# mjayantkumar/spark-timeseries

Measured on AMD Instinct MI355X. Metric: series-elements/sec + % HBM roofline (fill+lag+ACF) at 1/2/4/8 MI355X, higher is better.
Workload: dtype f64; 1 GPU; C3 shard: fill('linear') + autocorr(60), 12,500 series x 982,800 steps per GPU (N=8 -> C3's 100k x 982,800, 786 GB); series_per_gpu=12500, numLags=60, fill=linear, parallelism=dp1 (series sharded by key, one process per GPU)

## Files before the change

spark-timeseries_amd/csrc/sts_internal.hpp:

```cpp
#pragma once
#include <hip/hip_runtime.h>

#include <cstdint>
#include <cstdlib>

#include "sts.h"

namespace sts {

constexpr int kHB = 64;
constexpr int kHA = 128;
constexpr int kPartStride = 68;
constexpr int kPartSum = 64, kPartSq = 65, kPartShift = 66;
constexpr int kAcfEdge = 64;
constexpr bool kShortPairDefault = false;

struct TileArgs {
    const double* in;
    double* out;
    double* lagmat;
    double* partials;
    int32_t* err;
    int64_t S, T, ld_in, ld_out;
    int64_t tiles_per_series;
    int64_t tiles_per_chunk;
    int64_t chunks_per_series;
    int K;
    int max_lag;
    int include_original;
    double* acf_fused;
    const double* shift;
    int err_all;
};

struct FinalizeArgs {
    const double* F;
    const double* partials;
    double* acf;
    int64_t S, T, ldF, parts_per_series;
    int K;
    int32_t* exact;
};

#ifdef STS_AB
inline const char* ab_knob(const char* name) { return std::getenv(name); }
#else
inline const char* ab_knob(const char*) { return nullptr; }
#endif

int series_status(const int32_t* h, int64_t S, const char* what);
int set_error(int status, const char* msg);
int validate_call(int (*fn)(void*), void* ctx);
template <class F>
int validate(F&& f) {
    return validate_call([](void* c) { return (*static_cast<F*>(c))(); }, static_cast<void*>(&f));
}

hipError_t launch_tile(int method, int tw, const TileArgs& a, hipStream_t st);
hipError_t launch_acf_finalize(const FinalizeArgs& a, hipStream_t st);
hipError_t launch_acf_exact(const double* F, int64_t S, int64_t T, int64_t ldF, int K, const int32_t* exact,
                            double* acf, hipStream_t st);
hipError_t launch_acf_shift(const double* in, int64_t S, int64_t T, int64_t ld, int method, double* shift,
                            hipStream_t st);
constexpr int kFusedMaxLags = 63;
size_t acf_wide_partials(int64_t S, int64_t T, int K);
hipError_t launch_acf_wide(const double* F, int64_t S, int64_t T, int64_t ld, const double* shift, int K, double* part,
                           double* acf, int32_t* exact, hipStream_t st);

constexpr int kSegW = 512;
constexpr int kSegTiles = 128;
int seg_nt(int K);
hipError_t launch_segment(int method, const TileArgs& a, hipStream_t st);
bool short_ok(int method, int64_t T, int K);
hipError_t launch_short(int method, const TileArgs& a, hipStream_t st, bool pair);

int64_t spline_batch(int64_t S, int64_t T);
hipError_t launch_spline(const double* in, double* out, int64_t S, int64_t T, int64_t ld_in, int64_t ld_out,
                         int32_t* err, double* scratch, int64_t batch, hipStream_t st);

hipError_t launch_diff(const double* in, double* out, int64_t S, int64_t T, int64_t ld_in,
                       int64_t ld_out, int lag, int start, hipStream_t st);
hipError_t launch_diff_inplace(double* x, int64_t S, int64_t T, int64_t ld, int lag, int start,
                               hipStream_t st);
hipError_t launch_lagmat(const double* in, double* out, int64_t S, int64_t T, int64_t ld_in,
                         int max_lag, int include_original, hipStream_t st);
hipError_t launch_ewma_remove(const double* in, double* out, int64_t S, int64_t T, int64_t ld_in,
                              int64_t ld_out, const double* sm, hipStream_t st);
hipError_t launch_ar_remove(const double* in, double* out, int64_t S, int64_t T, int64_t ld_in,
                            int64_t ld_out, const double* c, const double* coef, int p,
                            hipStream_t st);

enum RecurOp { kEwmaAdd = 0, kEwmaRemoveInplace = 1, kArAdd = 2, kArRemoveInplace = 3,
               kFillDiffEwma = 4, kDiffInplace = 5 };
struct RecurArgs {
    const double* in;
    double* out;
    int64_t S, T, ld_in, ld_out;
    const double* sm;
    const double* c;
    const double* coef;
    int p;
    int lag, start;
    int method;
};
hipError_t launch_recur(RecurOp op, const RecurArgs& a, hipStream_t st);

struct ArArgs {
    const double* in;
    double* out;
    double* c;
    double* coef;
    int32_t* err;
    int64_t S, T, ld_in, ld_out;
    int p, no_intercept;
    int64_t* qr_list;
    uint32_t* qr_count;
};
hipError_t launch_ar_fit(const ArArgs& a, hipStream_t st);
hipError_t launch_ar_rule_count(const ArArgs& a, uint32_t* count, hipStream_t st);
bool ar_qr_lane_ok(int p);
size_t ar_qr_wave_slot_elems(int64_t T, int p, int no_intercept);
hipError_t launch_ar_qr(const ArArgs& a, const int64_t* list, const uint32_t* count, int64_t n_direct,
                        double* scratch, int slots, bool force_wave, hipStream_t st);

struct EwmaFitArgs {
    const double* in;
    int64_t S, T, ld;
    double* smoothing;
    double* sse;
    double* grad;
    int32_t* err;
    int32_t* evals;
};
hipError_t launch_ewma_fit(const EwmaFitArgs& a, bool fit, hipStream_t st);

struct GarchFitArgs {
    const double* in;
    int64_t S, T, ld;
    double* params;
    int32_t* err;
    int keep_err;
    int32_t* evals;
    double* loglik;
    double* grad;
    void* park;
    int64_t* park_ids;
    int32_t* park_ctr;
    int park_cap;
    int pass_budget;
};
hipError_t launch_garch_fit(const GarchFitArgs& a, bool fit, hipStream_t st);
enum GarchOp { kGarchRemove = 0, kGarchAdd = 1, kArgarchRemove = 2, kArgarchRemoveInplace = 3, kArgarchAdd = 4 };
struct GarchEffectsArgs {
    const double* in;
    double* out;
    int64_t S, T, ld_in, ld_out;
    const double *c, *phi, *omega, *alpha, *beta;
};
hipError_t launch_garch_effects(int op, const GarchEffectsArgs& a, hipStream_t st);

struct ArimaCssArgs {
    const double* in;
    int64_t S, ld;
    int n_len;
    int p, q, icpt;
    const double* coef_in;
    double* coef_out;
    int32_t* err;
    int32_t* evals;
    double* loglik;
    double* grad;
};
hipError_t launch_arima_css(const ArimaCssArgs& a, bool fit, hipStream_t st);
constexpr int kArimaChunk = 64;
enum ArimaOp { kArimaRemove = 0, kArimaAdd = 1, kArimaIntegrate = 2 };
struct ArimaEffectsArgs {
    const double* in;
    double* out;
    int64_t S, T, ld_in, ld_out;
    int p, q, icpt;
    const double* coef;
    int start;
};
hipError_t launch_arima_effects(int op, const ArimaEffectsArgs& a, hipStream_t st);
struct ArimaForecastArgs {
    const double* ts;
    const double* diffed;
    double* out;
    int64_t S, T, ld_ts, ld_d, ld_out;
    int d, n_future;
    int p, q, icpt;
    const double* coef;
};
hipError_t launch_arima_forecast(const ArimaForecastArgs& a, hipStream_t st);
hipError_t launch_arima_level_sum(const double* level, int64_t ld, double* sum, int64_t S, int64_t T, int first,
                                  hipStream_t st);
hipError_t launch_arima_diag(const double* level, int64_t ld, int64_t S, int64_t col, double* diag, int d, int k,
                             hipStream_t st);
hipError_t launch_arima_forecast_merge(const double* ts, int64_t ld_ts, const double* sum, const double* raw,
                                       const double* diag, double* out, int64_t ld_out, int64_t S, int64_t T, int d,
                                       int n_future, hipStream_t st);
struct ArimaHrArgs {
    const double* in;
    int64_t S, ld;
    int n_len;
    int p, q, icpt;
    const double* c;
    const double* phi;
    double* init_out;
    int32_t* err;
};
hipError_t launch_arima_hr(const ArimaHrArgs& a, hipStream_t st);

constexpr int64_t kStatOneWave = 2560;
struct StatArgs {
    const double* in;
    int64_t S, T, ld;
    double* stat;
    int32_t* err;
    int p;
    int q;
    int L;
};
hipError_t launch_dw(const StatArgs& a, hipStream_t st);
hipError_t launch_kpss(const StatArgs& a, hipStream_t st);
hipError_t launch_adf(const StatArgs& a, hipStream_t st);
hipError_t launch_adf_pvalue(const double* stat, double* pv, int64_t S, int regression, hipStream_t st);
hipError_t launch_lb(const double* acf, int64_t S, int64_t T, int K, double* stat, double* pv, hipStream_t st);
constexpr int kMaxFactors = STS_MAX_FACTORS;
struct BgBpArgs {
    const double* in;
    int64_t S, T, ld;
    const double* factors;
    int64_t ld_f, fs;
    int k;
    int L;
    bool squares;
    int64_t lo, n;
    double* basis;
    int64_t basis_stride;
    int32_t* info;
    int64_t info_stride;
    double* stat;
    int32_t* err;
};
bool own_basis(const BgBpArgs& a);
hipError_t launch_factor_basis(const BgBpArgs& a, int64_t s0, int64_t nb, hipStream_t st);
hipError_t launch_bgbp(const BgBpArgs& a, int64_t s0, int64_t ns, hipStream_t st);
hipError_t launch_chi2_pvalue(const double* stat, double* pv, int64_t S, int dof, hipStream_t st);

hipError_t launch_series_stats(const double* in, double* out, int64_t S, int64_t T, int64_t ld, hipStream_t st);
hipError_t launch_nan_instants(const double* in, uint8_t* flags, int64_t S, int64_t T, int64_t ld, hipStream_t st);
int64_t active_scratch_elems(int64_t T);
hipError_t launch_active_instants(const uint8_t* flags, int64_t T, int64_t* active, int64_t* n_active,
                                  int64_t* scratch, hipStream_t st);
hipError_t launch_gather_instants(const double* in, double* out, const int64_t* active, int64_t n_active, int64_t S,
                                  int64_t ld_in, int64_t ld_out, hipStream_t st);
hipError_t launch_transpose(const double* in, double* out, int64_t S, int64_t T, int64_t ld_in, int64_t ld_out,
                            hipStream_t st);

hipError_t launch_wire_decode(const unsigned char* bytes, const int64_t* val_off, double* panel, int64_t S, int64_t T,
                              int64_t ld, hipStream_t st);
hipError_t launch_wire_encode(const double* panel, int64_t S, int64_t T, int64_t ld, const int64_t* val_off,
                              unsigned char* bytes, hipStream_t st);
hipError_t launch_observations(const int32_t* sid, const int64_t* loc, const double* val, int64_t n, double* panel,
                               int64_t S, int64_t T, int64_t ld, unsigned char* win, hipStream_t st);

hipError_t launch_gen_panel(double* out, int64_t s0, int64_t S, int64_t T, int64_t ld,
                            uint64_t seed, uint32_t nan_thr, hipStream_t st);
hipError_t launch_gen_ar(double* out, double* c, double* phi, int64_t s0, int64_t S, int64_t T,
                         int64_t ld, uint64_t seed, int p, hipStream_t st);

}
```

spark-timeseries_amd/csrc/sts_tile.hip:

```cpp
#include "sts_internal.hpp"
#include "sts_lanes.hpp"
#include "sts_acf.hpp"
#include "sts_scan.hpp"

#include <hip/hip_runtime.h>

#include <type_traits>


#ifndef STS_FILL_PRIO
#define STS_FILL_PRIO 2
#endif
#ifndef STS_TILE_WGS
#define STS_TILE_WGS 4
#endif


namespace sts {
namespace {

__device__ __forceinline__ void lds_barrier() {
    __builtin_amdgcn_fence(__ATOMIC_RELEASE, "workgroup", "local");
    __builtin_amdgcn_s_barrier();
    __builtin_amdgcn_fence(__ATOMIC_ACQUIRE, "workgroup", "local");
}

typedef double d4 __attribute__((ext_vector_type(4)));
typedef double d2v __attribute__((ext_vector_type(2)));
typedef int i4v __attribute__((ext_vector_type(4)));

constexpr int kThreads = 256;
constexpr int kBig = 1 << 30;

#ifdef STS_STAMPS
__device__ unsigned long long g_stamps[16];
#define STAMP(i)                                                                            \
    do {                                                                                    \
        const unsigned long long now_ = __builtin_amdgcn_s_memtime();                      \
        st_acc[i] += now_ - st_prev;                                                        \
        st_prev = now_;                                                                     \
    } while (0)
#else
#define STAMP(i) \
    do {         \
    } while (0)
#endif

__device__ __forceinline__ int opq(int x) {
    asm volatile("" : "+v"(x));
    return x;
}

template <int L>
__device__ __forceinline__ void wlane(int& v, unsigned x) {
    asm("v_writelane_b32 %0, %1, %2" : "+v"(v) : "s"(x), "n"(L));
}

template <int CTRL>
__device__ __forceinline__ int dpp(int old, int v) {
    return __builtin_amdgcn_update_dpp(old, v, CTRL, 0xf, 0xf, false);
}
__device__ __forceinline__ int rl(int v, int l) { return __builtin_amdgcn_readlane(v, l); }
__device__ __forceinline__ int imax(int a, int b) { return a > b ? a : b; }
__device__ __forceinline__ int imin(int a, int b) { return a < b ? a : b; }
__device__ __forceinline__ int wave_prefix_max(int v, int lane) {
    constexpr int I = -0x7fffffff - 1;
    v = imax(v, dpp<0x111>(I, v));
    v = imax(v, dpp<0x112>(I, v));
    v = imax(v, dpp<0x114>(I, v));
    v = imax(v, dpp<0x118>(I, v));
    const int p1 = rl(v, 15), p2 = imax(p1, rl(v, 31)), p3 = imax(p2, rl(v, 47));
    const int r = opq(lane) >> 4;
    return imax(v, r == 0 ? I : r == 1 ? p1 : r == 2 ? p2 : p3);
}
__device__ __forceinline__ int wave_prefix_sum(int v, int lane) {
    v += dpp<0x111>(0, v);
    v += dpp<0x112>(0, v);
    v += dpp<0x114>(0, v);
    v += dpp<0x118>(0, v);
    const int p1 = rl(v, 15), p2 = p1 + rl(v, 31), p3 = p2 + rl(v, 47);
    const int r = opq(lane) >> 4;
    return v + (r == 0 ? 0 : r == 1 ? p1 : r == 2 ? p2 : p3);
}
__device__ __forceinline__ int wave_suffix_min(int v, int lane) {
    constexpr int I = 0x7fffffff;
    v = imin(v, dpp<0x101>(I, v));
    v = imin(v, dpp<0x102>(I, v));
    v = imin(v, dpp<0x104>(I, v));
    v = imin(v, dpp<0x108>(I, v));
    const int s3 = rl(v, 48), s2 = imin(s3, rl(v, 32)), s1 = imin(s2, rl(v, 16));
    const int r = opq(lane) >> 4;
    return imin(v, r == 0 ? s1 : r == 1 ? s2 : r == 2 ? s3 : I);
}

template <bool PAD>
__device__ __forceinline__ int px_(int q) { return PAD ? q + ((q >> 5) << 2) : q; }
template <bool PAD>
__device__ __forceinline__ int px2_(int q2) { return PAD ? q2 + ((q2 >> 4) << 1) : q2; }

template <int TW, int NT, bool SHIFTED, int NTH, int M>
__global__ __launch_bounds__(NTH, STS_TILE_WGS) void tile_kernel(TileArgs a) {
    constexpr int method = M;
    if constexpr (NT > 0) __builtin_amdgcn_s_setprio(STS_FILL_PRIO);
    constexpr int kThreads = NTH;
    constexpr int kWaves = NTH / 64;
    static_assert(TW / 64 % kWaves == 0, "whole 64-step chunks per wave");
    constexpr int EW = kHB + TW + kHA;
    constexpr int NA = SHIFTED ? 2 : (NT > 0 ? NT : 1);
    constexpr int QS = (SHIFTED && NT > 0) ? 16 / NT : 16;
    constexpr int REACH = (NT == 0) ? 0 : (SHIFTED ? 80 : 16 * NT);
    constexpr bool PAD = SHIFTED && NT > 0;
    constexpr int EWP = PAD ? EW + EW / 8 : EW;
    auto px = [](int q) { return px_<PAD>(q); };
    auto px2 = [](int q2) { return px2_<PAD>(q2); };
    constexpr int PX2S = PAD ? kThreads + 2 * (kThreads / 16) : kThreads;
    constexpr int PXW = PAD ? 72 : 64;
    static_assert(kThreads % 16 == 0, "linear padded strides");
    constexpr int NW = EW / 64;
    constexpr int NP2 = EW / 2;
    constexpr int RPT = (NP2 + kThreads - 1) / kThreads;
    static_assert(EW % 64 == 0, "extended tile must be whole words");
    static_assert(NW <= 128, "word scan handles at most 128 words");
    __shared__ __attribute__((aligned(16))) double vals[EWP];
    __shared__ unsigned long long mask[NW];
    __shared__ int lastUpTo[NW];
    __shared__ int firstFrom[NW];
    constexpr int NG = NW / 8 + 1;
    constexpr int NGQ = (NG + 3) / 4;
    __shared__ __attribute__((aligned(16))) int wbase[8 * NG];
    __shared__ __attribute__((aligned(16))) int wcoarse[4 * NGQ];
    __shared__ unsigned long long wneed[NW];
    __shared__ int sh_i[4];
    __shared__ double sh_d[3];
    __shared__ int carry_L[2], carry_t[2];
    __shared__ double carry_r[2];
    __shared__ int sh_c[4];

    const int tid = threadIdx.x;
    const int lane = tid & 63;
    const int wave = __builtin_amdgcn_readfirstlane(tid >> 6);
    const int64_t nchunk = a.S * a.chunks_per_series;
    const int64_t ch = xcd_remap(blockIdx.x, nchunk);
    const int64_t s = ch / a.chunks_per_series;
    const int64_t cidx = ch - s * a.chunks_per_series;
    const int64_t k_begin = cidx * a.tiles_per_chunk;
    const int64_t k_end = (k_begin + a.tiles_per_chunk < a.tiles_per_series) ? k_begin + a.tiles_per_chunk
                                                                              : a.tiles_per_series;
    const int64_t T = a.T;
    const double* src = a.in + s * a.ld_in;
    const bool src_al = (reinterpret_cast<uintptr_t>(src) & 15) == 0;
    constexpr bool needL = (method == STS_FILL_LINEAR || method == STS_FILL_PREVIOUS || method == STS_FILL_NEAREST);
    constexpr bool needN = (method == STS_FILL_LINEAR || method == STS_FILL_NEXT || method == STS_FILL_NEAREST);
    double* dst = a.out ? a.out + s * a.ld_out : nullptr;
    const int64_t lrows = T - a.max_lag;
    const int ncols = a.max_lag + (a.include_original ? 1 : 0);
    const int init = a.include_original ? 0 : 1;

    if (tid < 2) {
        carry_L[tid] = -1;
        carry_t[tid] = -kBig;
    }
    if (tid == 0) {
        sh_c[0] = -kBig;
        sh_c[2] = -1;
    }
    if (tid < 8) {
        if (NW + 1 + tid < 8 * NG) wbase[NW + 1 + tid] = kBig;
        if (NG + tid < 4 * NGQ) wcoarse[NG + tid] = kBig;
    }
    double acc_s = 0.0, acc_q = 0.0;

    static_assert(RPT <= 9, "prefetch registers are spelled out for RPT <= 9");
    double2 R0, R1, R2, R3, R4, R5, R6, R7, R8;
    auto interior = [&](int64_t kk) {
        const int64_t e0 = kk * TW - kHB;
        return e0 >= 0 && e0 + EW <= T && src_al;
    };
#define STS_LD1(j)                                                                          \
    if constexpr (j < RPT) {                                                                \
        const int q2_ = tid + j * kThreads;                                                 \
        const double2* p_ = &s2_[q2_ < NP2 ? q2_ : NP2 - 1];                                \
        if constexpr (NT > 0) {                                                             \
            const d2v v_ = __builtin_nontemporal_load(reinterpret_cast<const d2v*>(p_));    \
            R##j = make_double2(v_.x, v_.y);                                                \
        } else {                                                                            \
            R##j = *p_;                                                                     \
        }                                                                                   \
    }
#define STS_ISSUE(kk)                                                                       \
    do {                                                                                    \
        const double2* s2_ = reinterpret_cast<const double2*>(src + ((kk) * TW - kHB));     \
        STS_LD1(0) STS_LD1(1) STS_LD1(2) STS_LD1(3) STS_LD1(4)                              \
        STS_LD1(5) STS_LD1(6) STS_LD1(7) STS_LD1(8)                                         \
    } while (0)
#define STS_CLEAR()                                                                         \
    do {                                                                                    \
        asm volatile("" : "=v"(R0), "=v"(R1), "=v"(R2), "=v"(R3), "=v"(R4));               \
        asm volatile("" : "=v"(R5), "=v"(R6), "=v"(R7), "=v"(R8));                         \
    } while (0)
#define STS_ST1(j)                                                                          \
    if constexpr (j < RPT) {                                                                \
        const int q2_ = tid + j * kThreads;                                                 \
        if ((j + 1) * kThreads <= NP2 || q2_ < NP2) v2_[pst_ + j * PX2S] = R##j;            \
    }

    d4 U[NA];
#pragma unroll
    for (int t = 0; t < NA; t++) U[t] = d4{0.0, 0.0, 0.0, 0.0};
    bool series_err = false;
#ifdef STS_STAMPS
    unsigned long long st_acc[12] = {0};
    unsigned long long st_prev = __builtin_amdgcn_s_memtime();
#endif
    bool have = interior(k_begin);
    if (have) STS_ISSUE(k_begin);
    else STS_CLEAR();
    const double c0 = [&] {
        if constexpr (NT == 0) return 0.0;
        const double v = a.shift[s];
        const unsigned long long u = __builtin_bit_cast(unsigned long long, v);
        const unsigned lo = __builtin_amdgcn_readfirstlane((unsigned)u);
        const unsigned hi = __builtin_amdgcn_readfirstlane((unsigned)(u >> 32));
        return __builtin_bit_cast(double, ((unsigned long long)hi << 32) | lo);
    }();

    constexpr int qA0 = kHB;
    constexpr int NTA = NT > 0 ? NT : 1;
    constexpr int CPW = TW / 64 / kWaves;
    auto mid_sums = [&](int p, double y) {
        const double z = acf_mid(p + lane, T) ? y : 0.0;
        acc_s += z;
        acc_q = __builtin_fma(z, z, acc_q);
    };
    auto mfma_group = [&](auto FROM, auto TO, const double* vb, int64_t kk, int tt0, int tt1) {
        constexpr int F = decltype(FROM)::value, TE = decltype(TO)::value;
        if constexpr (NT > 0 && F < TE) {
            const bool tile_mid = tt0 >= kAcfEdge && tt1 + kAcfEdge <= T;
            const int tlen = tt1 - tt0;
            const int nch = (tlen + 63) / 64;
            const bool full = wave * CPW + CPW <= nch;
            int c = wave * CPW + F;
            int cend = wave * CPW + TE;
            if (cend > nch) cend = nch;
            if constexpr (SHIFTED) {
                int oa[NTA], ob[NTA];
#pragma unroll
                for (int t = 0; t < NT; t++) {
                    const int j = lane & 15;
                    const int ra = QS * t + lane;
                    const int rb = QS * t + 16 * (lane >> 4) + 16 * (j / QS) + (16 - QS) + (j % QS);
                    oa[t] = opq(px(ra));
                    ob[t] = opq(px(rb));
                }
                auto chunk_mfma = [&](const double* yb) {
                    double av[NTA], bv[NTA];
#pragma unroll
                    for (int t = 0; t < NT; t++) {
                        av[t] = yb[oa[t]];
                        bv[t] = yb[ob[t]];
                    }
#pragma unroll
                    for (int t = 0; t < NT; t++)
                        U[t % NA] = __builtin_amdgcn_mfma_f64_16x16x4f64(av[t], bv[t], U[t % NA], 0, 0, 0);
                    return av[0];
                };
                if (F == 0 && kk == 0 && wave == 0) chunk_mfma(vb);
                if (full && tile_mid) {
                    int ia[NTA], ib[NTA];
                    const int cb = px(qA0 + 64 * (wave * CPW));
#pragma unroll
                    for (int t = 0; t < NT; t++) {
                        ia[t] = cb + oa[t];
                        ib[t] = cb + ob[t];
                        asm volatile("" : "+v"(ia[t]), "+v"(ib[t]));
                    }
#pragma unroll
                    for (int cc = F; cc < TE; cc++) {
                        double av[NTA], bv[NTA];
#pragma unroll
                        for (int t = 0; t < NT; t++) {
                            av[t] = vb[ia[t] + 72 * cc];
                            bv[t] = vb[ib[t] + 72 * cc];
                        }
#pragma unroll
                        for (int t = 0; t < NT; t++)
                            U[t % NA] = __builtin_amdgcn_mfma_f64_16x16x4f64(av[t], bv[t], U[t % NA], 0, 0, 0);
                        acc_s += av[0];
                        acc_q = __builtin_fma(av[0], av[0], acc_q);
                        __builtin_amdgcn_sched_barrier(0);
                    }
                    c = cend;
                }
                for (; c < cend; c++) mid_sums(tt0 + 64 * c, chunk_mfma(vb + px(qA0 + 64 * c)));
            } else {
                for (; c < cend; c++) {
                    const int jrel = 64 * c + lane;
                    double bv[NTA];
#pragma unroll
                    for (int t = 0; t < NT; t++) bv[t] = vb[px(qA0 + jrel + 16 * t)];
                    const double av = (jrel < tlen) ? bv[0] : 0.0;
#pragma unroll
                    for (int t = 0; t < NT; t++) U[t] = __builtin_amdgcn_mfma_f64_16x16x4f64(av, bv[t], U[t], 0, 0, 0);
                    mid_sums(tt0 + 64 * c, av);
                }
            }
        }
    };
    for (int64_t k = k_begin; k < k_end; k++) {
        const int t0 = (int)(k * TW);
        const int t1 = (t0 + TW < T) ? t0 + TW : (int)T;
        const int e0 = t0 - kHB;

        if (have) {
            double2* v2_ = reinterpret_cast<double2*>(vals);
            const int pst_ = opq(px2(tid));
            STS_ST1(0) STS_ST1(1) STS_ST1(2) STS_ST1(3) STS_ST1(4) STS_ST1(5) STS_ST1(6) STS_ST1(7) STS_ST1(8)
#define STS_BAL1(j)                                                                         \
    if constexpr (j < RPT) {                                                                \
        const unsigned long long bx_ = __ballot(!isnan_d(R##j.x));                          \
        const unsigned long long by_ = __ballot(!isnan_d(R##j.y));                          \
        const unsigned long long lo_ = interleave2((unsigned)bx_, (unsigned)by_);           \
        const unsigned long long hi_ = interleave2((unsigned)(bx_ >> 32), (unsigned)(by_ >> 32)); \
        wlane<4 * j + 0>(mv_, (unsigned)lo_);                                               \
        wlane<4 * j + 1>(mv_, (unsigned)(lo_ >> 32));                                       \
        wlane<4 * j + 2>(mv_, (unsigned)hi_);                                               \
        wlane<4 * j + 3>(mv_, (unsigned)(hi_ >> 32));                                       \
    }
            {
                int mv_ = 0;
                STS_BAL1(0) STS_BAL1(1) STS_BAL1(2) STS_BAL1(3) STS_BAL1(4) STS_BAL1(5) STS_BAL1(6)
                STS_BAL1(7) STS_BAL1(8)
                const int w_ = 2 * wave + 2 * kWaves * (lane >> 2) + ((lane >> 1) & 1);
                if (lane < 4 * RPT && w_ < NW) reinterpret_cast<int*>(mask)[2 * w_ + (lane & 1)] = mv_;
            }
#undef STS_BAL1
        } else {
            for (int q = tid; q < EW; q += kThreads) {
                const int t = e0 + q;
                vals[px(q)] = (t >= 0 && t < T) ? src[t] : __builtin_nan("");
            }
        }
        const bool have_next = (k + 1 < k_end) && interior(k + 1);
        STAMP(0);
        lds_barrier();
        STAMP(1);

        const int qA = kHB;
        const int qW = kHB + (t1 - t0);
        int qB = qW + REACH;
        if (e0 + qB > T) qB = (int)T - e0;

        if (!have) {
            const int pb = opq(px(lane) + PXW * wave);
#pragma unroll 1
            for (int i = 0; i < (NW + kWaves - 1) / kWaves; i++) {
                const int w = wave + i * kWaves;
                if (w < NW) {
                    const unsigned long long m = __ballot(!isnan_d(vals[pb + PXW * kWaves * i]));
                    if (lane == 0) mask[w] = m;
                }
            }
            STAMP(2);
            lds_barrier();
        }
        STAMP(3);

        if (wave == 0) {
            if constexpr (NT > 0) __builtin_amdgcn_s_setprio(3);
            int w0 = 2 * lane;
            asm volatile("" : "+v"(w0));
            const int w1 = w0 + 1;
            const unsigned long long m0 = (w0 < NW) ? mask[w0] : ~0ull;
            const unsigned long long m1 = (w1 < NW) ? mask[w1] : ~0ull;
            const int l0 = (w0 < NW && m0) ? w0 * 64 + 63 - __clzll(m0) : -1;
            const int l1 = (w1 < NW && m1) ? w1 * 64 + 63 - __clzll(m1) : -1;
            const int f0 = (w0 < NW && m0) ? w0 * 64 + __ffsll(m0) - 1 : kBig;
            const int f1 = (w1 < NW && m1) ? w1 * 64 + __ffsll(m1) - 1 : kBig;
            auto need = [&](int w, unsigned long long m) -> unsigned long long {
                const int lo = qA - w * 64, hi = qB - w * 64;
                if (method == STS_FILL_NONE || hi <= 0 || lo >= 64) return 0ull;
                unsigned long long r = ~m;
                if (lo > 0) r &= ~0ull << lo;
                if (hi < 64) r &= (1ull << hi) - 1ull;
                return r;
            };
            const unsigned long long n0 = (w0 < NW) ? need(w0, m0) : 0ull;
            const unsigned long long n1 = (w1 < NW) ? need(w1, m1) : 0ull;
            const int pm = wave_prefix_max(l1 > l0 ? l1 : l0, lane);
            const int sm = wave_suffix_min(f0 < f1 ? f0 : f1, lane);
            const int pc = wave_prefix_sum(__popcll(n0) + __popcll(n1), lane);
            const int ex = dpp<0x138>(-1, pm);
            const int exc = dpp<0x138>(0, pc);
            const int exs = dpp<0x130>(kBig, sm);
            const int nnan = rl(pc, 63);
            const int firstValidE = rl(sm, 0);
            const int lastValidE = rl(pm, 63);
            const bool lg = method == STS_FILL_LINEAR &&
                            __ballot((w0 < NW && __popcll(~m0) > kLongRun / 2) ||
                                     (w1 < NW && __popcll(~m1) > kLongRun / 2)) != 0ull;
            if (w0 < NW) {
                lastUpTo[w0] = ex > l0 ? ex : l0;
                const int a0 = f1 < exs ? f1 : exs;
                firstFrom[w0] = f0 < a0 ? f0 : a0;
                wbase[w0] = exc;
                wneed[w0] = n0;
                if ((lane & 3) == 0) wcoarse[lane >> 2] = exc;
            }
            if (w1 < NW) {
                const int a1 = ex > l0 ? ex : l0;
                lastUpTo[w1] = a1 > l1 ? a1 : l1;
                firstFrom[w1] = f1 < exs ? f1 : exs;
                wbase[w1] = exc + __popcll(n0);
                wneed[w1] = n1;
            }
            int lext = -1, next = (int)T;
            if (needL && e0 > 0 && firstValidE > qA && nnan > 0)
                lext = (sh_c[0] == e0) ? sh_c[1] : (int)scan_back(src, e0, lane);
            if (needN && e0 + EW < T && qB > qA && lastValidE < qB - 1 && nnan > 0) {
                const int from = e0 + EW;
                const int cN_pos = sh_c[2], cN = sh_c[3];
                next = (cN_pos >= 0 && cN_pos <= from && cN >= from) ? cN : (int)scan_fwd(src, from, T, lane);
                if (lane == 0) {
                    sh_c[2] = from;
                    sh_c[3] = next;
                }
            }
            if (needL) {
                const int lq = rl(pm, TW / 128 - 1);
                if (lane == 0) {
                    sh_c[0] = e0 + TW;
                    sh_c[1] = (lq >= 0) ? e0 + lq : lext;
                }
            }
            if (lane == 0) {
                wbase[NW] = nnan;
                if constexpr (NW % 8 == 0) wcoarse[NW / 8] = nnan;
                sh_i[0] = lext;
                sh_i[1] = next;
                sh_i[2] = nnan;
                sh_i[3] = lg ? 1 : 0;
            }
            if (lext >= 0) {
                const double v = src[lext];
                if (lane == 0) sh_d[1] = v;
            }
            if (next < T) {
                const double v = src[next];
                if (lane == 0) sh_d[2] = v;
            }
        }
        if constexpr (NT > 0) __builtin_amdgcn_s_setprio(STS_FILL_PRIO);
        STAMP(4);
        lds_barrier();
        STAMP(5);

        {
            const int nnan = sh_i[2];
            const int lext = sh_i[0], next = sh_i[1];
            const double lextv = sh_d[1], nextv = sh_d[2];
            auto impute = [&](auto long_tag) {
            constexpr bool LONG = decltype(long_tag)::value;
            for (int idx = tid; idx < nnan; idx += kThreads) {
                const i4v* c4 = reinterpret_cast<const i4v*>(wcoarse);
                int g = -1;
#pragma unroll
                for (int j = 0; j < NGQ; j++) {
                    const i4v c = c4[j];
                    g += (c.x <= idx) + (c.y <= idx) + (c.z <= idx) + (c.w <= idx);
                }
                const i4v* b4 = reinterpret_cast<const i4v*>(wbase) + 2 * g;
                const i4v ba = b4[0], bb = b4[1];
                const int w = 8 * g - 1 + (ba.x <= idx) + (ba.y <= idx) + (ba.z <= idx) + (ba.w <= idx) +
                              (bb.x <= idx) + (bb.y <= idx) + (bb.z <= idx) + (bb.w <= idx);
                unsigned long long nm = wneed[w];
                const int wb = wbase[w];
                const unsigned long long m = mask[w];
                const int lup = needL ? lastUpTo[w > 0 ? w - 1 : 0] : -1;
                const int ffr = needN ? firstFrom[w + 1 < NW ? w + 1 : NW - 1] : kBig;
                int kk = idx - wb, b = 0;
#pragma unroll
                for (int width = 32; width >= 1; width >>= 1) {
                    const int c = __popcll(nm & ((1ull << width) - 1ull));
                    if (kk >= c) { kk -= c; nm >>= width; b += width; }
                }
                const int q = w * 64 + b;
                const int t = e0 + q;
                int Lt = -1, Nt = (int)T;
                double Lv = 0.0, Nv = 0.0;
                if (needL) {
                    const unsigned long long lo = m & ((1ull << b) - 1ull);
                    const int Lq = lo ? w * 64 + 63 - __clzll(lo) : (w > 0 ? lup : -1);
                    if (Lq >= 0) { Lt = e0 + Lq; Lv = vals[px(Lq)]; }
                    else { Lt = lext; Lv = lextv; }
                }
                if (needN) {
                    const unsigned long long hi = (b == 63) ? 0ull : (m & (~0ull << (b + 1)));
                    const int Nq = hi ? w * 64 + __ffsll(hi) - 1 : (w + 1 < NW ? ffr : kBig);
                    if (Nq < kBig) { Nt = e0 + Nq; Nv = vals[px(Nq)]; }
                    else { Nt = next; Nv = nextv; }
                }
                double f = __builtin_nan("");
                switch (method) {
                case STS_FILL_PREVIOUS:
                    if (Lt >= 0) f = Lv;
                    break;
                case STS_FILL_NEXT:
                    if (Nt < T) f = Nv;
                    break;
                case STS_FILL_NEAREST: {
                    if (t == 0) break;
                    const int P = (Lt >= 1) ? Lt : -1;
                    if (P < 0 && Nt >= T) { series_err = true; break; }
                    f = (Nt >= T || (P >= 0 && t - P < Nt - t)) ? Lv : Nv;
                    break;
                }
                case STS_FILL_LINEAR: {
                    if (Lt < 0 || Nt >= T) break;
                    if (LONG && t - Lt > kLongRun) {
                        if (t - Lt == kLongRun + 1 || q == qA) {
                            const double inc = (Nv - Lv) / (double)(Nt - Lt);
                            const int rd = (int)((k + 1) & 1), wr = (int)(k & 1);
                            double v;
                            if (carry_L[rd] == Lt && carry_t[rd] == t - 1) {
                                v = carry_r[rd];
                            } else {
                                v = Lv;
                                int j = t - 1 - Lt;
                                for (; j >= 8; j -= 8) {
                                    v = v + inc; v = v + inc; v = v + inc; v = v + inc;
                                    v = v + inc; v = v + inc; v = v + inc; v = v + inc;
                                }
                                for (; j > 0; j--) v = v + inc;
                            }
                            const int qend = (Nt - e0 < qB) ? Nt - e0 : qB;
                            for (int qq = q; qq < qend; qq++) {
                                v = v + inc;
                                vals[px(qq)] = v;
                                if (e0 + qq == t1 - 1) {
                                    carry_L[wr] = Lt;
                                    carry_t[wr] = t1 - 1;
                                    carry_r[wr] = v;
                                }
                            }
                        }
                        continue;
                    }
                    const double inc = (Nv - Lv) / (double)(Nt - Lt);
                    double r = Lv;
                    for (int j = t - Lt; j > 0; j--) r = r + inc;
                    f = r;
                    break;
                }
                default:
                    break;
                }
                vals[px(q)] = f;
            }
        };
            if (sh_i[3]) impute(std::true_type{});
            else impute(std::false_type{});
        }
        STAMP(6);
        lds_barrier();
        STAMP(7);

        {
            const bool al = dst && ((reinterpret_cast<uintptr_t>(dst) & 15) == 0);
            double2* v2 = reinterpret_cast<double2*>(vals);
            const int qBfull = (NT > 0) ? ((SHIFTED || qW + 64 + 16 * NT >= EW) ? EW : qW + 64 + 16 * NT) : 0;
            const bool fast = (dst == nullptr || al) && (t1 - t0 == TW) && (NT == 0 || e0 + qW + REACH <= T);
            if (fast) {
                constexpr int FS = TW / 2 / kThreads;
                constexpr int FY = NT > 0 ? (NP2 - kHB / 2 + kThreads - 1) / kThreads : FS;
                constexpr int FH = (FY + 1) / 2;
                const int vq = (kHB >> 1) + tid;
                const int pvq = opq(px2(vq));
                const bool wr = dst != nullptr;
                char* const dpb = reinterpret_cast<char*>(dst + t0);
                unsigned dpo = (unsigned)tid * 16u;
                asm volatile("" : "+v"(dpo));
#pragma unroll
                for (int h = 0; h < 2; h++) {
                    double2 fv[FH];
#pragma unroll
                    for (int j = 0; j < FH; j++) {
                        const int jj = h * FH + j;
                        if (jj < FY && (jj * kThreads + kThreads <= NP2 - kHB / 2 ||
                                        tid + jj * kThreads < NP2 - kHB / 2))
                            fv[j] = v2[pvq + jj * PX2S];
                    }
#pragma unroll
                    for (int j = 0; j < FH; j++) {
                        const int jj = h * FH + j;
                        if (jj >= FY) continue;
                        const bool in = jj * kThreads + kThreads <= NP2 - kHB / 2 ||
                                        tid + jj * kThreads < NP2 - kHB / 2;
                        if (jj < FS && wr) {
                            double2* dq = reinterpret_cast<double2*>(dpb + jj * kThreads * 16 + dpo);
                            __builtin_nontemporal_store(fv[j].x, &dq->x);
                            __builtin_nontemporal_store(fv[j].y, &dq->y);
                        }
                        if (NT > 0 && in) {
                            double2 y;
                            y.x = fv[j].x - c0;
                            y.y = fv[j].y - c0;
                            v2[pvq + jj * PX2S] = y;
                        }
                    }
                }
            } else
            for (int q2 = (qA >> 1) + tid; 2 * q2 < qW || 2 * q2 < qBfull; q2 += kThreads) {
                const int q = 2 * q2;
                double2 f = v2[px2(q2)];
                if (q < qW) {
                    const int t = e0 + q;
                    if (dst) {
                        if (al && q + 1 < qW) {
                            *reinterpret_cast<double2*>(dst + t) = f;
                        } else {
                            dst[t] = f.x;
                            if (q + 1 < qW) dst[t + 1] = f.y;
                        }
                    }
                }
                if (NT > 0 && q < qBfull) {
                    f.x = (q < qB) ? f.x - c0 : 0.0;
                    f.y = (q + 1 < qB) ? f.y - c0 : 0.0;
                    v2[px2(q2)] = f;
                }
            }
            if (SHIFTED && NT > 0 && e0 < 0 && tid < kHB / 2) v2[px2(tid)] = make_double2(0.0, 0.0);
        }
        if (have_next) STS_ISSUE(k + 1);
        else STS_CLEAR();
        if constexpr (NT == 0) {
            if (a.lagmat) {
                double* lm = a.lagmat + s * lrows * ncols;
                for (int c = init; c <= a.max_lag; c++) {
                    double* col = lm + (int64_t)(c - init) * lrows;
                    const int sh = a.max_lag - c;
                    const int rlo = t0 - sh > 0 ? t0 - sh : 0;
                    const int rhi = (int64_t)(t1 - sh) < lrows ? t1 - sh : (int)lrows;
                    if (rlo >= rhi) continue;
                    const int par = (int)((reinterpret_cast<uintptr_t>(col) >> 3) & 1);
                    const int rp = rlo - ((rlo + par) & 1);
                    for (int r = rp + 2 * tid; r < rhi; r += 2 * kThreads) {
                        const int q = r + sh - e0;
                        if (r >= rlo && r + 1 < rhi) {
                            *reinterpret_cast<d2v*>(col + r) = d2v{vals[px(q)], vals[px(q + 1)]};
                        } else {
                            if (r >= rlo) col[r] = vals[px(q)];
                            if (r + 1 < rhi) col[r + 1] = vals[px(q + 1)];
                        }
                    }
                }
            }
        }
        STAMP(8);

        if constexpr (NT > 0) {
            lds_barrier();
            STAMP(9);
            __builtin_amdgcn_s_setprio(0);
            mfma_group(std::integral_constant<int, 0>{}, std::integral_constant<int, CPW>{}, vals, k, t0, t1);
            __builtin_amdgcn_s_setprio(STS_FILL_PRIO);
        }
        have = have_next;
        STAMP(10);
        lds_barrier();
        STAMP(11);
    }
#undef STS_ISSUE
#undef STS_LD1
#undef STS_ST1
#undef STS_CLEAR
    if (series_err && a.err) a.err[s] = STS_ERR_ALL_NAN;
#ifdef STS_STAMPS
    if (lane == 0) {
#pragma unroll
        for (int i = 0; i < 12; i++) atomicAdd(&g_stamps[i], st_acc[i]);
        atomicAdd(&g_stamps[12], 1ull);
    }
#endif

    if constexpr (NT > 0) {
        double* scr = vals + wave * 256;
        double lagacc = 0.0;
        if constexpr (SHIFTED) {
            d4 D = U[0];
#pragma unroll
            for (int t = 1; t < NA; t++) D += U[t];
#pragma unroll
            for (int r = 0; r < 4; r++) scr[((lane >> 4) + 4 * r) * 16 + (lane & 15)] = D[r];
            lds_barrier();
#pragma unroll
            for (int j = 0; j < 16; j++) {
                const int i = 16 * (j / QS) + (16 - QS) + (j % QS) - lane;
                if (i >= 0 && i < 16) lagacc += scr[i * 16 + j];
            }
            lds_barrier();
        } else {
#pragma unroll
            for (int t = 0; t < NT; t++) {
#pragma unroll
                for (int r = 0; r < 4; r++) scr[((lane >> 4) + 4 * r) * 16 + (lane & 15)] = U[t][r];
                lds_barrier();
#pragma unroll
                for (int b = 0; b < 16; b++)
                    if (((b + lane) >> 4) == t) lagacc += scr[b * 16 + ((b + lane) & 15)];
                lds_barrier();
            }
        }
#pragma unroll
        for (int d = 32; d >= 1; d >>= 1) {
            acc_s += __shfl_xor(acc_s, d);
            acc_q += __shfl_xor(acc_q, d);
        }
        double* wsum = vals + kWaves * 256;
        wsum[wave * kPartStride + lane] = lagacc;
        if (lane == 0) {
            wsum[wave * kPartStride + kPartSum] = acc_s;
            wsum[wave * kPartStride + kPartSq] = acc_q;
        }
        lds_barrier();
        if (wave == 0) {
            double* part = a.partials + ch * kPartStride;
            double tot = 0.0;
#pragma unroll
            for (int w = 0; w < kWaves; w++) tot += wsum[w * kPartStride + lane];
            part[lane] = tot;
            if (lane == 0) {
                double ts = 0.0, tq = 0.0;
#pragma unroll
                for (int w = 0; w < kWaves; w++) {
                    ts += wsum[w * kPartStride + kPartSum];
                    tq += wsum[w * kPartStride + kPartSq];
                }
                part[kPartSum] = ts;
                part[kPartSq] = tq;
                part[kPartShift] = c0;
            }
        }
    }
}

__global__ __launch_bounds__(256) void acf_finalize_kernel(FinalizeArgs a) {
    const int lane = threadIdx.x & 63;
    const int64_t s = (int64_t)blockIdx.x * 4 + (threadIdx.x >> 6);
    if (s >= a.S) return;
    const int K = a.K;
    const int i = lane + 1;
    const int64_t T = a.T;
    const double* F = a.F + s * a.ldF;
    if (lane >= K) return;
    double out;
    if (i >= T) {
        out = __builtin_nan("");
    } else if (T <= 2 * (int64_t)K || T < 2 * kAcfEdge) {
        out = acf_exact_lag(F, T, i);
    } else {
        double Pi = 0.0, Sm = 0.0, Qm = 0.0;
        const double* pp = a.partials + s * a.parts_per_series * kPartStride;
        const double c = pp[kPartShift];
        for (int64_t k = 0; k < a.parts_per_series; k++, pp += kPartStride) {
            Pi += pp[i];
            Sm += pp[kPartSum];
            Qm += pp[kPartSq];
        }
        bool sus;
        out = acf_combine(Pi, Sm, Qm, i, T, [&](int j) { return F[j] - c; },
                          [&](int j) { return F[T - 1 - j] - c; }, c, &sus);
        if (__ballot(sus) && lane == 0) a.exact[s] = 1;
    }
    a.acf[s * K + lane] = out;
}

constexpr int kExactChunk = 512;
template <bool WIDE>
__global__ __launch_bounds__(256) void acf_exact_kernel(const double* __restrict__ F, int64_t S, int64_t T,
                                                        int64_t ld, int K, int nblk, const int32_t* __restrict__ flags,
                                                        double* __restrict__ acf) {
    __shared__ double lds[4][kExactChunk + 64];
    __shared__ double ldsb[4][WIDE ? kExactChunk : 1];
    const int wave = threadIdx.x >> 6, lane = threadIdx.x & 63;
    const int nb = WIDE ? nblk - 1 : 1;
    const int64_t u = (int64_t)blockIdx.x * 4 + wave;
    const int64_t s = u / nb;
    if (s >= S || !flags[s]) return;
    const int b = WIDE ? 1 + (int)(u % nb) : 0;
    const int i = b * 64 + lane + 1;
    const bool active = i <= K && (int64_t)i < T;
    const double r = WIDE ? acf_exact_stream<kExactChunk, true>(F + s * ld, T, i, active, lds[wave], lane, b * 64,
                                                                ldsb[wave])
                          : acf_exact_stream<kExactChunk>(F + s * ld, T, i, active, lds[wave], lane);
    if (active) acf[s * K + (i - 1)] = r;
}

__global__ __launch_bounds__(256) void acf_shift_kernel(const double* in, int64_t S, int64_t T, int64_t ld, int prev,
                                                        double* shift) {
    const int lane = threadIdx.x & 63;
    const int64_t s = (int64_t)blockIdx.x * 4 + (threadIdx.x >> 6);
    if (s >= S) return;
    const double c = robust_shift(in + s * ld, T, lane, prev != 0);
    if (lane == 0) shift[s] = c;
}

}

hipError_t launch_acf_shift(const double* in, int64_t S, int64_t T, int64_t ld, int method, double* shift,
                            hipStream_t st) {
    if (S <= 0 || T <= 0) return hipSuccess;
    dim3 grid((unsigned)((S + 3) / 4)), block(256);
    hipLaunchKernelGGL(acf_shift_kernel, grid, block, 0, st, in, S, T, ld, method == STS_FILL_PREVIOUS ? 1 : 0,
                       shift);
    return hipGetLastError();
}

template <int TW, int NT, bool SHIFTED, int NTH>
hipError_t launch_m(int method, dim3 grid, const TileArgs& a, hipStream_t st) {
    const dim3 block(NTH);
    switch (method) {
    case STS_FILL_NONE: hipLaunchKernelGGL((tile_kernel<TW, NT, SHIFTED, NTH, STS_FILL_NONE>), grid, block, 0, st, a); break;
    case STS_FILL_LINEAR: hipLaunchKernelGGL((tile_kernel<TW, NT, SHIFTED, NTH, STS_FILL_LINEAR>), grid, block, 0, st, a); break;
    case STS_FILL_NEAREST: hipLaunchKernelGGL((tile_kernel<TW, NT, SHIFTED, NTH, STS_FILL_NEAREST>), grid, block, 0, st, a); break;
    case STS_FILL_NEXT: hipLaunchKernelGGL((tile_kernel<TW, NT, SHIFTED, NTH, STS_FILL_NEXT>), grid, block, 0, st, a); break;
    case STS_FILL_PREVIOUS: hipLaunchKernelGGL((tile_kernel<TW, NT, SHIFTED, NTH, STS_FILL_PREVIOUS>), grid, block, 0, st, a); break;
    default: return hipErrorInvalidValue;
    }
    return hipGetLastError();
}

hipError_t launch_tile(int method, int tw, const TileArgs& a, hipStream_t st) {
    const int64_t nchunk = a.S * a.chunks_per_series;
    if (nchunk <= 0) return hipSuccess;
    if (nchunk > 0x7fffffffLL) return hipErrorInvalidValue;
    dim3 grid((unsigned)nchunk);
    if (tw == 512 && a.K == 0) return launch_m<512, 0, false, kThreads>(method, grid, a, st);
#ifdef STS_AB
    if (tw == 2048 && a.K > 0 && a.K <= 60) {
        if (a.K <= 24) return launch_m<2048, 2, true, kThreads / 2>(method, grid, a, st);
        return launch_m<2048, 4, true, kThreads / 2>(method, grid, a, st);
    }
#endif
    if (tw != 4096) return hipErrorInvalidValue;
    if (a.K == 0) return launch_m<4096, 0, false, kThreads>(method, grid, a, st);
    if (a.K <= 24) return launch_m<4096, 2, true, kThreads>(method, grid, a, st);
    if (a.K <= 60) return launch_m<4096, 4, true, kThreads>(method, grid, a, st);
    if (a.K <= 63) return launch_m<4096, 5, false, kThreads>(method, grid, a, st);
    return hipErrorInvalidValue;
}

#ifdef STS_STAMPS
extern "C" int sts_debug_stamps(unsigned long long* out16) {
    if (hipMemcpyFromSymbol(out16, HIP_SYMBOL(g_stamps), sizeof(unsigned long long) * 16) != hipSuccess) return 4;
    unsigned long long z[16] = {0};
    return hipMemcpyToSymbol(HIP_SYMBOL(g_stamps), z, sizeof(z)) == hipSuccess ? 0 : 4;
}
#endif

hipError_t launch_acf_finalize(const FinalizeArgs& a, hipStream_t st) {
    if (a.S <= 0 || a.K <= 0) return hipSuccess;
    dim3 grid((unsigned)((a.S + 3) / 4)), block(256);
    hipLaunchKernelGGL(acf_finalize_kernel, grid, block, 0, st, a);
    return hipGetLastError();
}

hipError_t launch_acf_exact(const double* F, int64_t S, int64_t T, int64_t ldF, int K, const int32_t* exact,
                            double* acf, hipStream_t st) {
    if (S <= 0 || K <= 0 || T <= 0) return hipSuccess;
    const int nblk = (K + 63) / 64;
    if ((S * nblk + 3) / 4 > 0x7fffffffLL) return hipErrorInvalidValue;
    hipLaunchKernelGGL(acf_exact_kernel<false>, dim3((unsigned)((S + 3) / 4)), dim3(256), 0, st, F, S, T, ldF, K, nblk,
                       exact, acf);
    hipError_t e = hipGetLastError();
    if (e != hipSuccess || nblk == 1) return e;
    hipLaunchKernelGGL(acf_exact_kernel<true>, dim3((unsigned)((S * (nblk - 1) + 3) / 4)), dim3(256), 0, st, F, S, T,
                       ldF, K, nblk, exact, acf);
    return hipGetLastError();
}

}
```

Measured before the change: 300.1 billion series-elements/s.

## Carry tile overlap in registers instead of re-reading back halo from HBM

For the ACF path (NT>0), the back halo (HB) is set to zero. The 128-step forward halo of each tile is kept in R8 and written into the start of the next tile's LDS buffer, so input is no longer re-read from global memory for the overlap. The last valid position and value for linear fill are carried across tiles in shared memory, which replaces the scan_back lookups. The first tile's mask and MFMA boundary handling get special cases. This cuts redundant HBM reads, in exchange for more intricate cross-iteration state and a higher risk of correctness bugs.

```diff
diff --git a/spark-timeseries_amd/csrc/sts_internal.hpp b/spark-timeseries_amd/csrc/sts_internal.hpp
--- a/spark-timeseries_amd/csrc/sts_internal.hpp
+++ b/spark-timeseries_amd/csrc/sts_internal.hpp
@@ -10,6 +10,7 @@
 
 constexpr int kHB = 64;
 constexpr int kHA = 128;
+constexpr int kHBCarry = 0;
 constexpr int kPartStride = 68;
 constexpr int kPartSum = 64, kPartSq = 65, kPartShift = 66;
 constexpr int kAcfEdge = 64;
diff --git a/spark-timeseries_amd/csrc/sts_tile.hip b/spark-timeseries_amd/csrc/sts_tile.hip
--- a/spark-timeseries_amd/csrc/sts_tile.hip
+++ b/spark-timeseries_amd/csrc/sts_tile.hip
@@ -105,7 +105,9 @@
     constexpr int kThreads = NTH;
     constexpr int kWaves = NTH / 64;
     static_assert(TW / 64 % kWaves == 0, "whole 64-step chunks per wave");
-    constexpr int EW = kHB + TW + kHA;
+    constexpr bool CARRY = NT > 0;
+    constexpr int HB = CARRY ? kHBCarry : kHB;
+    constexpr int EW = HB + TW + kHA;
     constexpr int NA = SHIFTED ? 2 : (NT > 0 ? NT : 1);
     constexpr int QS = (SHIFTED && NT > 0) ? 16 / NT : 16;
     constexpr int REACH = (NT == 0) ? 0 : (SHIFTED ? 80 : 16 * NT);
@@ -118,7 +120,11 @@
     static_assert(kThreads % 16 == 0, "linear padded strides");
     constexpr int NW = EW / 64;
     constexpr int NP2 = EW / 2;
-    constexpr int RPT = (NP2 + kThreads - 1) / kThreads;
+    constexpr int LOFF2 = CARRY ? kHA / 2 : 0;
+    constexpr int NPM = NP2 - LOFF2;
+    constexpr int RPT = (NPM + kThreads - 1) / kThreads;
+    static_assert(!CARRY || (NPM == 8 * kThreads && kHA == 128 && LOFF2 % 16 == 0),
+                  "CARRY: eight full registers, and the handed-on steps fill R8 of one wave");
     static_assert(EW % 64 == 0, "extended tile must be whole words");
     static_assert(NW <= 128, "word scan handles at most 128 words");
     __shared__ __attribute__((aligned(16))) double vals[EWP];
@@ -135,6 +141,8 @@
     __shared__ int carry_L[2], carry_t[2];
     __shared__ double carry_r[2];
     __shared__ int sh_c[4];
+    __shared__ int cpos;
+    __shared__ double cval;
 
     const int tid = threadIdx.x;
     const int lane = tid & 63;
@@ -163,6 +171,10 @@
     if (tid == 0) {
         sh_c[0] = -kBig;
         sh_c[2] = -1;
+        if constexpr (CARRY) {
+            cpos = -1;
+            cval = 0.0;
+        }
     }
     if (tid < 8) {
         if (NW + 1 + tid < 8 * NG) wbase[NW + 1 + tid] = kBig;
@@ -173,13 +185,13 @@
     static_assert(RPT <= 9, "prefetch registers are spelled out for RPT <= 9");
     double2 R0, R1, R2, R3, R4, R5, R6, R7, R8;
     auto interior = [&](int64_t kk) {
-        const int64_t e0 = kk * TW - kHB;
+        const int64_t e0 = kk * TW - HB;
         return e0 >= 0 && e0 + EW <= T && src_al;
     };
 #define STS_LD1(j)                                                                          \
     if constexpr (j < RPT) {                                                                \
         const int q2_ = tid + j * kThreads;                                                 \
-        const double2* p_ = &s2_[q2_ < NP2 ? q2_ : NP2 - 1];                                \
+        const double2* p_ = &s2_[LOFF2 + (((j + 1) * kThreads <= NPM || q2_ < NPM) ? q2_ : NPM - 1)]; \
         if constexpr (NT > 0) {                                                             \
             const d2v v_ = __builtin_nontemporal_load(reinterpret_cast<const d2v*>(p_));    \
             R##j = make_double2(v_.x, v_.y);                                                \
@@ -189,9 +201,15 @@
     }
 #define STS_ISSUE(kk)                                                                       \
     do {                                                                                    \
-        const double2* s2_ = reinterpret_cast<const double2*>(src + ((kk) * TW - kHB));     \
+        const double2* s2_ = reinterpret_cast<const double2*>(src + ((kk) * TW - HB));      \
         STS_LD1(0) STS_LD1(1) STS_LD1(2) STS_LD1(3) STS_LD1(4)                              \
         STS_LD1(5) STS_LD1(6) STS_LD1(7) STS_LD1(8)                                         \
+    } while (0)
+#define STS_ISSUE_HEAD(kk)                                                                  \
+    do {                                                                                    \
+        const d2v* h2_ = reinterpret_cast<const d2v*>(src + (kk) * TW);                     \
+        const d2v v_ = __builtin_nontemporal_load(&h2_[tid & 63]);                          \
+        R8 = make_double2(v_.x, v_.y);                                                      \
     } while (0)
 #define STS_CLEAR()                                                                         \
     do {                                                                                    \
@@ -201,7 +219,7 @@
 #define STS_ST1(j)                                                                          \
     if constexpr (j < RPT) {                                                                \
         const int q2_ = tid + j * kThreads;                                                 \
-        if ((j + 1) * kThreads <= NP2 || q2_ < NP2) v2_[pst_ + j * PX2S] = R##j;            \
+        if ((j + 1) * kThreads <= NPM || q2_ < NPM) v2_[pst_ + j * PX2S] = R##j;            \
     }
 
     d4 U[NA];
@@ -213,8 +231,12 @@
     unsigned long long st_prev = __builtin_amdgcn_s_memtime();
 #endif
     bool have = interior(k_begin);
-    if (have) STS_ISSUE(k_begin);
-    else STS_CLEAR();
+    if (have) {
+        STS_ISSUE(k_begin);
+        if constexpr (CARRY) STS_ISSUE_HEAD(k_begin);
+    } else {
+        STS_CLEAR();
+    }
     const double c0 = [&] {
         if constexpr (NT == 0) return 0.0;
         const double v = a.shift[s];
@@ -224,7 +246,7 @@
         return __builtin_bit_cast(double, ((unsigned long long)hi << 32) | lo);
     }();
 
-    constexpr int qA0 = kHB;
+    constexpr int qA0 = HB;
     constexpr int NTA = NT > 0 ? NT : 1;
     constexpr int CPW = TW / 64 / kWaves;
     auto mid_sums = [&](int p, double y) {
@@ -264,7 +286,21 @@
                         U[t % NA] = __builtin_amdgcn_mfma_f64_16x16x4f64(av[t], bv[t], U[t % NA], 0, 0, 0);
                     return av[0];
                 };
-                if (F == 0 && kk == 0 && wave == 0) chunk_mfma(vb);
+                if (F == 0 && kk == 0 && wave == 0) {
+                    double av[NTA], bv[NTA];
+#pragma unroll
+                    for (int t = 0; t < NT; t++) {
+                        const int j = lane & 15;
+                        const bool ina = QS * t + lane >= 64;
+                        const bool inb = QS * t + 16 * (lane >> 4) + 16 * (j / QS) + (16 - QS) + (j % QS) >= 64;
+                        const double ya = vb[ina ? oa[t] - 72 : 0], yb = vb[inb ? ob[t] - 72 : 0];
+                        av[t] = ina ? ya : 0.0;
+                        bv[t] = inb ? yb : 0.0;
+                    }
+#pragma unroll
+                    for (int t = 0; t < NT; t++)
+                        U[t % NA] = __builtin_amdgcn_mfma_f64_16x16x4f64(av[t], bv[t], U[t % NA], 0, 0, 0);
+                }
                 if (full && tile_mid) {
                     int ia[NTA], ib[NTA];
                     const int cb = px(qA0 + 64 * (wave * CPW));
@@ -306,15 +342,29 @@
             }
         }
     };
+    bool carried = false;
     for (int64_t k = k_begin; k < k_end; k++) {
         const int t0 = (int)(k * TW);
         const int t1 = (t0 + TW < T) ? t0 + TW : (int)T;
-        const int e0 = t0 - kHB;
+        const int e0 = t0 - HB;
 
         if (have) {
             double2* v2_ = reinterpret_cast<double2*>(vals);
-            const int pst_ = opq(px2(tid));
+            const int pst_ = opq(px2(LOFF2 + tid));
             STS_ST1(0) STS_ST1(1) STS_ST1(2) STS_ST1(3) STS_ST1(4) STS_ST1(5) STS_ST1(6) STS_ST1(7) STS_ST1(8)
+            if constexpr (CARRY) {
+                if (wave == 0) {
+                    v2_[pst_ - px2(LOFF2)] = R8;
+                    if (!carried) {
+                        const unsigned long long bx = __ballot(!isnan_d(R8.x));
+                        const unsigned long long by = __ballot(!isnan_d(R8.y));
+                        if (lane == 0) {
+                            mask[0] = interleave2((unsigned)bx, (unsigned)by);
+                            mask[1] = interleave2((unsigned)(bx >> 32), (unsigned)(by >> 32));
+                        }
+                    }
+                }
+            }
 #define STS_BAL1(j)                                                                         \
     if constexpr (j < RPT) {                                                                \
         const unsigned long long bx_ = __ballot(!isnan_d(R##j.x));                          \
@@ -330,7 +380,7 @@
                 int mv_ = 0;
                 STS_BAL1(0) STS_BAL1(1) STS_BAL1(2) STS_BAL1(3) STS_BAL1(4) STS_BAL1(5) STS_BAL1(6)
                 STS_BAL1(7) STS_BAL1(8)
-                const int w_ = 2 * wave + 2 * kWaves * (lane >> 2) + ((lane >> 1) & 1);
+                const int w_ = LOFF2 / 32 + 2 * wave + 2 * kWaves * (lane >> 2) + ((lane >> 1) & 1);
                 if (lane < 4 * RPT && w_ < NW) reinterpret_cast<int*>(mask)[2 * w_ + (lane & 1)] = mv_;
             }
 #undef STS_BAL1
@@ -345,8 +395,8 @@
         lds_barrier();
         STAMP(1);
 
-        const int qA = kHB;
-        const int qW = kHB + (t1 - t0);
+        const int qA = HB;
+        const int qW = HB + (t1 - t0);
         int qB = qW + REACH;
         if (e0 + qB > T) qB = (int)T - e0;
 
@@ -372,6 +422,8 @@
             const int w1 = w0 + 1;
             const unsigned long long m0 = (w0 < NW) ? mask[w0] : ~0ull;
             const unsigned long long m1 = (w1 < NW) ? mask[w1] : ~0ull;
+            const int cpos_in = CARRY ? cpos : -1;
+            const double cval_in = CARRY ? cval : 0.0;
             const int l0 = (w0 < NW && m0) ? w0 * 64 + 63 - __clzll(m0) : -1;
             const int l1 = (w1 < NW && m1) ? w1 * 64 + 63 - __clzll(m1) : -1;
             const int f0 = (w0 < NW && m0) ? w0 * 64 + __ffsll(m0) - 1 : kBig;
@@ -395,9 +447,9 @@
             const int nnan = rl(pc, 63);
             const int firstValidE = rl(sm, 0);
             const int lastValidE = rl(pm, 63);
-            const bool lg = method == STS_FILL_LINEAR &&
-                            __ballot((w0 < NW && __popcll(~m0) > kLongRun / 2) ||
-                                     (w1 < NW && __popcll(~m1) > kLongRun / 2)) != 0ull;
+            bool lg = method == STS_FILL_LINEAR &&
+                      __ballot((w0 < NW && __popcll(~m0) > kLongRun / 2) ||
+                               (w1 < NW && __popcll(~m1) > kLongRun / 2)) != 0ull;
             if (w0 < NW) {
                 lastUpTo[w0] = ex > l0 ? ex : l0;
                 const int a0 = f1 < exs ? f1 : exs;
@@ -414,8 +466,14 @@
                 wneed[w1] = n1;
             }
             int lext = -1, next = (int)T;
-            if (needL && e0 > 0 && firstValidE > qA && nnan > 0)
-                lext = (sh_c[0] == e0) ? sh_c[1] : (int)scan_back(src, e0, lane);
+            if constexpr (CARRY) {
+                if (carried) lext = cpos_in;
+                else if (needL && e0 > 0 && firstValidE > qA && nnan > 0) lext = (int)scan_back(src, e0, lane);
+                if (method == STS_FILL_LINEAR && firstValidE > qA && lext >= 0 && e0 - lext > kLongRun / 2) lg = true;
+            } else {
+                if (needL && e0 > 0 && firstValidE > qA && nnan > 0)
+                    lext = (sh_c[0] == e0) ? sh_c[1] : (int)scan_back(src, e0, lane);
+            }
             if (needN && e0 + EW < T && qB > qA && lastValidE < qB - 1 && nnan > 0) {
                 const int from = e0 + EW;
                 const int cN_pos = sh_c[2], cN = sh_c[3];
@@ -425,11 +483,18 @@
                     sh_c[3] = next;
                 }
             }
-            if (needL) {
-                const int lq = rl(pm, TW / 128 - 1);
+            const int lq = rl(pm, TW / 128 - 1);
+            if (needL && !CARRY) {
                 if (lane == 0) {
                     sh_c[0] = e0 + TW;
                     sh_c[1] = (lq >= 0) ? e0 + lq : lext;
+                }
+            }
+            if (needL && CARRY && lq >= 0) {
+                const double v = vals[px(lq)];
+                if (lane == 0) {
+                    cpos = e0 + lq;
+                    cval = v;
                 }
             }
             if (lane == 0) {
@@ -440,9 +505,17 @@
                 sh_i[2] = nnan;
                 sh_i[3] = lg ? 1 : 0;
             }
-            if (lext >= 0) {
+            if (CARRY && carried) {
+                if (lane == 0) sh_d[1] = cval_in;
+            } else if (lext >= 0) {
                 const double v = src[lext];
-                if (lane == 0) sh_d[1] = v;
+                if (lane == 0) {
+                    sh_d[1] = v;
+                    if (CARRY && lq < 0) {
+                        cpos = lext;
+                        cval = v;
+                    }
+                }
             }
             if (next < T) {
                 const double v = src[next];
@@ -571,9 +644,9 @@
             const bool fast = (dst == nullptr || al) && (t1 - t0 == TW) && (NT == 0 || e0 + qW + REACH <= T);
             if (fast) {
                 constexpr int FS = TW / 2 / kThreads;
-                constexpr int FY = NT > 0 ? (NP2 - kHB / 2 + kThreads - 1) / kThreads : FS;
+                constexpr int FY = NT > 0 ? (NP2 - HB / 2 + kThreads - 1) / kThreads : FS;
                 constexpr int FH = (FY + 1) / 2;
-                const int vq = (kHB >> 1) + tid;
+                const int vq = (HB >> 1) + tid;
                 const int pvq = opq(px2(vq));
                 const bool wr = dst != nullptr;
                 char* const dpb = reinterpret_cast<char*>(dst + t0);
@@ -585,16 +658,17 @@
 #pragma unroll
                     for (int j = 0; j < FH; j++) {
                         const int jj = h * FH + j;
-                        if (jj < FY && (jj * kThreads + kThreads <= NP2 - kHB / 2 ||
-                                        tid + jj * kThreads < NP2 - kHB / 2))
+                        if (jj < FY && (jj * kThreads + kThreads <= NP2 - HB / 2 ||
+                                        tid + jj * kThreads < NP2 - HB / 2))
                             fv[j] = v2[pvq + jj * PX2S];
                     }
 #pragma unroll
                     for (int j = 0; j < FH; j++) {
                         const int jj = h * FH + j;
                         if (jj >= FY) continue;
-                        const bool in = jj * kThreads + kThreads <= NP2 - kHB / 2 ||
-                                        tid + jj * kThreads < NP2 - kHB / 2;
+                        const bool in = jj * kThreads + kThreads <= NP2 - HB / 2 ||
+                                        tid + jj * kThreads < NP2 - HB / 2;
+                        if (CARRY && jj == FS) R8 = fv[j];
                         if (jj < FS && wr) {
                             double2* dq = reinterpret_cast<double2*>(dpb + jj * kThreads * 16 + dpo);
                             __builtin_nontemporal_store(fv[j].x, &dq->x);
@@ -608,29 +682,31 @@
                         }
                     }
                 }
-            } else
-            for (int q2 = (qA >> 1) + tid; 2 * q2 < qW || 2 * q2 < qBfull; q2 += kThreads) {
-                const int q = 2 * q2;
-                double2 f = v2[px2(q2)];
-                if (q < qW) {
-                    const int t = e0 + q;
-                    if (dst) {
-                        if (al && q + 1 < qW) {
-                            *reinterpret_cast<double2*>(dst + t) = f;
-                        } else {
-                            dst[t] = f.x;
-                            if (q + 1 < qW) dst[t + 1] = f.y;
+            } else {
+                if constexpr (CARRY) R8 = v2[opq(px2(TW / 2 + (tid & 63)))];
+                for (int q2 = (qA >> 1) + tid; 2 * q2 < qW || 2 * q2 < qBfull; q2 += kThreads) {
+                    const int q = 2 * q2;
+                    double2 f = v2[px2(q2)];
+                    if (q < qW) {
+                        const int t = e0 + q;
+                        if (dst) {
+                            if (al && q + 1 < qW) {
+                                *reinterpret_cast<double2*>(dst + t) = f;
+                            } else {
+                                dst[t] = f.x;
+                                if (q + 1 < qW) dst[t + 1] = f.y;
+                            }
                         }
                     }
-                }
-                if (NT > 0 && q < qBfull) {
-                    f.x = (q < qB) ? f.x - c0 : 0.0;
-                    f.y = (q + 1 < qB) ? f.y - c0 : 0.0;
-                    v2[px2(q2)] = f;
-                }
-            }
-            if (SHIFTED && NT > 0 && e0 < 0 && tid < kHB / 2) v2[px2(tid)] = make_double2(0.0, 0.0);
-        }
+                    if (NT > 0 && q < qBfull) {
+                        f.x = (q < qB) ? f.x - c0 : 0.0;
+                        f.y = (q + 1 < qB) ? f.y - c0 : 0.0;
+                        v2[px2(q2)] = f;
+                    }
+                }
+            }
+        }
+        if (CARRY && have_next && tid < 2) mask[tid] = mask[NW - 2 + tid];
         if (have_next) STS_ISSUE(k + 1);
         else STS_CLEAR();
         if constexpr (NT == 0) {
@@ -666,11 +742,13 @@
             __builtin_amdgcn_s_setprio(STS_FILL_PRIO);
         }
         have = have_next;
+        carried = true;
         STAMP(10);
         lds_barrier();
         STAMP(11);
     }
 #undef STS_ISSUE
+#undef STS_ISSUE_HEAD
 #undef STS_LD1
 #undef STS_ST1
 #undef STS_CLEAR
```

Measured after the change: 301.4 billion series-elements/s, median of 6. No clear change (+0.4%).
